# CompVis/behavior-driven-video-synthesis

Hardware: AMD Instinct MI355X
Metric: frames/sec VUnet 256x256 bs=16 fwd+bwd (higher is better)
Workload: dtype f32 (operands scaled by a power of two and split into 2 fp16 terms, 3 partial products on fp16 MFMA, fp32 accumulate; weight gradients and uncovered layers: 3 bf16 terms / 6 products, fp32-input MFMA, fp32 VALU); 1 GPU; Human3.6m shape_and_pose_net VunetAlter 256x256 per-GPU bs=16 fwd+bwd, VGG19 perceptual + KL loss, fused Adam, dropout 0.05, regressor side loop off, seeded-synthetic VGG19 weights, rasterised synthetic stickmen; global_batch=16, parallelism=dp1, conv_precision=h2, hip_streams=4, hip_graph=True, graph_settle_steps=7, rccl_world_size=1, dp_backend=none

## Files before the change

behavior_driven_video_synthesis_amd/csrc/conv_p2.hip:

```cpp
#include <stdio.h>

#include <type_traits>

#include "common.h"
#include "split_h2.h"

namespace {

constexpr int P2_META = 128, P2_AMAX0 = 16, P2_NSLOT = 64;

struct P2Args {
  const uint4* x;
  const int* xmeta;
  const uint4* w;
  const float* wk;
  const float* shift;
  const uint4* mask;
  uint4* y;
  int* ymeta;
  int N, C, H, W, M;
  int relu;
};

__device__ __forceinline__ void p2_dma(uint32_t voff, const void* sbase, uint32_t lds_addr) {
// ... 284 lines not shown
  for (size_t i = (size_t)blockIdx.x * 256 + threadIdx.x; i < total; i += (size_t)gridDim.x * 256) {
    const int xw = (int)(i % W);
    size_t t = i / W;
    const int yh = (int)(t % H);
    t /= H;
    const float* src = x + (t * 8) * HW + (size_t)yh * W + xw;
    float v[8];
#pragma unroll
    for (int j = 0; j < 8; ++j) {
      float f = src[j * HW];
      if (relu) f = f > 0.f ? f : 0.f;
      v[j] = f * s;
    }
    uint4 h, l;
    h2_split2(v[0], v[1], h.x, l.x);
    h2_split2(v[2], v[3], h.y, l.y);
    h2_split2(v[4], v[5], h.z, l.z);
    h2_split2(v[6], v[7], h.w, l.w);
    const size_t o = (t * Hp + (yh + 1)) * Wp + (xw + 1);
    y[o] = h;
    y[plane + o] = l;
  }
}
__device__ __forceinline__ void p2_unpack(const uint4& h, const uint4& l, float inv, float* v) {
  const uint32_t hs[4] = {h.x, h.y, h.z, h.w}, ls[4] = {l.x, l.y, l.z, l.w};
#pragma unroll
  for (int j = 0; j < 4; ++j) {
    const h2_f16x2 a = __builtin_bit_cast(h2_f16x2, hs[j]), b = __builtin_bit_cast(h2_f16x2, ls[j]);
    v[2 * j] = ((float)a[0] + (float)b[0] * (1.f / 2048.f)) * inv;
    v[2 * j + 1] = ((float)a[1] + (float)b[1] * (1.f / 2048.f)) * inv;
  }
}
__global__ __launch_bounds__(256) void p2_to_nchw_kernel(const uint4* __restrict__ x, const int* __restrict__ xmeta,
                                                         float* __restrict__ y, int N, int C, int H, int W) {
  const int CB = C >> 3, Hp = H + 2, Wp = W + 2;
  const float inv = h2_pow2(-xmeta[0]);
  const size_t HW = (size_t)H * W, total = (size_t)N * CB * HW, plane = (size_t)N * CB * Hp * Wp;
  for (size_t i = (size_t)blockIdx.x * 256 + threadIdx.x; i < total; i += (size_t)gridDim.x * 256) {
    const int xw = (int)(i % W);
    size_t t = i / W;
    const int yh = (int)(t % H);
    t /= H;
    const size_t o = (t * Hp + (yh + 1)) * Wp + (xw + 1);
    float v[8];
    p2_unpack(x[o], x[plane + o], inv, v);
    float* dst = y + (t * 8) * HW + (size_t)yh * W + xw;
#pragma unroll
    for (int j = 0; j < 8; ++j) dst[j * HW] = v[j];
  }
}
}

extern "C" int vunet_p2_from_nchw(const float* x, const float* amax, int32_t n_amax, int32_t relu, void* y, int32_t* ymeta,
                                  int32_t N, int32_t C, int32_t H, int32_t W, void* stream) {
  if (!x || !amax || n_amax < 1 || !y || !ymeta || C % 8 || N < 1) return VUNET_ERR_ARG;
// ... 19 lines not shown
```

behavior_driven_video_synthesis_amd/csrc/conv_thin.hip:

```cpp
#include <string.h>

#include "conv_route.h"
#include "split_h2.h"

template <int MODE>
__global__ __launch_bounds__(256) void conv_thin_m_kernel(const GatherArgs a) {
  const vunet_conv_desc& d = a.d;
  const int H = d.Hs, W = d.Ws, HW = a.HsWs;
  const int tiles_w = (W + 31) / 32, tiles_h = (H + 7) / 8;
  const unsigned bid = xcd_remap(blockIdx.x, gridDim.x);
  const int tx = bid % tiles_w;
  const int ty = (bid / tiles_w) % tiles_h;
  const int n = bid / (tiles_w * tiles_h);
  const int ow = tx * 32 + (threadIdx.x & 31), oh = ty * 8 + (threadIdx.x >> 5);
  const bool inside = ow < W && oh < H;
  int off[9];
  uint32_t ok = 0;
#pragma unroll
  for (int t = 0; t < 9; ++t) {
    const int ih = oh + t / 3 - 1, iw = ow + t % 3 - 1;
    const bool v = inside && (unsigned)ih < (unsigned)H && (unsigned)iw < (unsigned)W;
    off[t] = v ? ih * W + iw : 0;
    ok |= (v ? 1u : 0u) << t;
  }
// ... 76 lines not shown
    for (int t = 0; t < 9; ++t) {
      const int tap = MODE == 0 ? t : 8 - t;
      const float* __restrict__ w = wt + (size_t)(tap * Cp + c) * d.Mpad;
#pragma unroll
      for (int r = 0; r < R; ++r)
#pragma unroll
        for (int m = 0; m < 4; ++m) acc[r][m] = fmaf(w[m], xv[r + t / 3][t % 3], acc[r][m]);
    }
  }
  if (ow >= W) return;
  PixGeo g;
  g.n = n;
  g.ow = ow;
  g.valid = true;
#pragma unroll
  for (int r = 0; r < R; ++r) {
    g.oh = oh0 + r;
    if (g.oh < H) {
#pragma unroll
      for (int m = 0; m < 4; ++m)
        if (m < d.M) store_out(a, g, m, acc[r][m]);
    }
  }
}

template <int KS, int CI>
__global__ __launch_bounds__(256, KS == 3 ? 2 : 4) void conv_thin_k_kernel(const GatherArgs a) {
  constexpr int T = KS * KS;
  const vunet_conv_desc& d = a.d;
  const int H = d.Hs, W = d.Ws, HW = a.HsWs;
  const int tiles_w = (W + 31) / 32, tiles_h = (H + 7) / 8;
  const unsigned bid = xcd_remap(blockIdx.x, gridDim.x);
  const int tx = bid % tiles_w;
  const int ty = (bid / tiles_w) % tiles_h;
  const int n = bid / (tiles_w * tiles_h);
  const int ow = tx * 32 + (threadIdx.x & 31), oh = ty * 8 + (threadIdx.x >> 5);
  const bool inside = ow < W && oh < H;
  constexpr int C = CI, Cp = (C + 1) & ~1;
  float xv[CI][T];
  const float* __restrict__ xs = a.x1 + (size_t)n * C * HW;
#pragma unroll
  for (int t = 0; t < T; ++t) {
    const int ih = oh + (KS == 3 ? t / 3 - 1 : 0), iw = ow + (KS == 3 ? t % 3 - 1 : 0);
    const bool v = inside && (unsigned)ih < (unsigned)H && (unsigned)iw < (unsigned)W;
    const int off = v ? ih * W + iw : 0;
#pragma unroll
// ... 226 lines not shown
    else VUNET_LAUNCH((conv_thin_k_kernel<1, 3>), grid, block, 0, st, ga);
  }
  return vunet_check_launch();
}

extern "C" int vunet_p2_conv_first(const float* x, const float* amax_x, int32_t n_amax, const float* wt_f, int32_t Mpad,
                                   const float* shift, const float* wk, void* y, int32_t* ymeta, int32_t N, int32_t H, int32_t W,
                                   int32_t M, void* stream) {
  if (!x || !amax_x || n_amax < 1 || !wt_f || !wk || !y || !ymeta) return VUNET_ERR_ARG;
  if (N < 1 || M < 8 || M % 8 || M > 128 || H % 32 || W % 32 || ((uintptr_t)y & 15)) return VUNET_ERR_UNSUPPORTED;
  GatherArgs ga;
  memset(&ga, 0, sizeof(ga));
  vunet_conv_desc& d = ga.d;
  d.N = N; d.C1 = 3; d.C2 = 0; d.Hs = H; d.Ws = W; d.M = M; d.m_off = 0; d.Mpad = Mpad; d.Ho = H; d.Wo = W; d.KH = 3; d.KW = 3;
  d.stride = 1; d.pad = 1; d.mode = 0; d.out_act = ACT_RELU;
  ga.x1 = x; ga.wt = wt_f; ga.shift = shift; ga.y = reinterpret_cast<float*>(y);
  ga.NP = N * H * W; ga.HoWo = H * W; ga.HsWs = H * W;
  ga.ph = ga.pw = -1;
  P2Out po{amax_x, (int)n_amax, wk, (int*)ymeta};
  dim3 gv((unsigned)(N * (H / 32) * (W / 32)));
  VUNET_LAUNCH((conv_thin_kv_kernel<3, 4, true>), gv, dim3(256), 0, (hipStream_t)stream, ga, po);
  return vunet_check_launch();
}
```

behavior_driven_video_synthesis_amd/csrc/conv_wgrad_thin.hip:

```cpp
#include "common.h"
#include "conv_wgrad_route.h"

struct WgradThinArgs {
  vunet_wgrad_desc d;
  const float* x1;
  const float* dy;
  float* slabs;
  float* dshift;
  int Coutp, tiles_w, tiles_per_img, ntiles;
  InAct in1;
};

__global__ __launch_bounds__(256) void conv_wgrad_thin_kernel(const WgradThinArgs a_in) {
  WgradThinArgs a = a_in;
  inact_resolve(a.in1);
  constexpr int TH = 8, TW = 32, IH = TH + 2, IW = TW + 3;
  const vunet_wgrad_desc& d = a.d;
  const int C = d.C1, H = d.Hs, W = d.Ws, HW = H * W;
  const int CP = IH * IW + 1;
  extern __shared__ __attribute__((aligned(16))) float smem[];
  float* const xT = smem;
  float4* const dyT = reinterpret_cast<float4*>(smem + ((C * CP + 3) & ~3));
  const int tid = threadIdx.x;
  const int nitems = 3 * C;
  int G = 1;
  while (G < 8 && 2 * G * nitems <= 256) G *= 2;
  const int RG = TH / G;
  const int grp = tid / nitems, it = tid - grp * nitems;
  const bool worker = grp < G;
  const int kh = it / C, ci = it - kh * C;

  float acc[3][4];
#pragma unroll
  for (int kw = 0; kw < 3; ++kw)
#pragma unroll
    for (int c = 0; c < 4; ++c) acc[kw][c] = 0.f;
  float dpart[4] = {0.f, 0.f, 0.f, 0.f};
  const int sg = tid / (TW + 2), scol = tid - sg * (TW + 2);

  for (int tile = blockIdx.x; tile < a.ntiles; tile += gridDim.x) {
    const int n = tile / a.tiles_per_img, tr = tile - n * a.tiles_per_img;
    const int ty = tr / a.tiles_w, tx = tr - ty * a.tiles_w;
    const int row0 = ty * TH, col0 = tx * TW;
    __syncthreads();
    if (sg < 7) {
      const int iw = col0 - 1 + scol;
      const bool cok = (unsigned)iw < (unsigned)W;
      for (int p0 = sg; p0 < C * IH; p0 += 7 * 8) {
        float v[8];
        uint32_t idx[8];
        bool ok[8];
#pragma unroll
        for (int e = 0; e < 8; ++e) {
          const int p = p0 + 7 * e;
          const int c = p / IH, r = p - c * IH;
          const int ih = row0 - 1 + r;
          ok[e] = p < C * IH && cok && (unsigned)ih < (unsigned)H;
          idx[e] = ok[e] ? (uint32_t)((n * C + c) * HW + ih * W + iw) : 0u;
          v[e] = a.x1[idx[e]];
        }
#pragma unroll
        for (int e = 0; e < 8; ++e) {
          const int p = p0 + 7 * e;
          if (p < C * IH) {
            const int c = p / IH, r = p - c * IH;
            xT[c * CP + r * IW + scol] = ok[e] ? apply_in_act(a.in1, v[e], idx[e]) : 0.f;
          }
        }
      }
    }
    {
      const int r = tid >> 5, col = tid & 31;
      float v[4] = {0.f, 0.f, 0.f, 0.f};
#pragma unroll
      for (int co = 0; co < 4; ++co)
        if (co < d.Cout) v[co] = a.dy[(size_t)(n * d.Cout + co) * HW + (row0 + r) * W + col0 + col];
      dyT[tid] = make_float4(v[0], v[1], v[2], v[3]);
#pragma unroll
      for (int co = 0; co < 4; ++co) dpart[co] += v[co];
    }
    __syncthreads();
    if (worker) {
      for (int rr = 0; rr < RG; ++rr) {
        const int r = grp * RG + rr;
        const float* xp = xT + ci * CP + (r + kh) * IW;
        float x0 = xp[0], x1 = xp[1];
#pragma unroll 8
        for (int col = 0; col < TW; ++col) {
          const float x2 = xp[col + 2];
          const float4 g = dyT[r * TW + col];
          acc[0][0] = fmaf(g.x, x0, acc[0][0]);
          acc[0][1] = fmaf(g.y, x0, acc[0][1]);
          acc[0][2] = fmaf(g.z, x0, acc[0][2]);
          acc[0][3] = fmaf(g.w, x0, acc[0][3]);
          acc[1][0] = fmaf(g.x, x1, acc[1][0]);
          acc[1][1] = fmaf(g.y, x1, acc[1][1]);
          acc[1][2] = fmaf(g.z, x1, acc[1][2]);
          acc[1][3] = fmaf(g.w, x1, acc[1][3]);
          acc[2][0] = fmaf(g.x, x2, acc[2][0]);
          acc[2][1] = fmaf(g.y, x2, acc[2][1]);
          acc[2][2] = fmaf(g.z, x2, acc[2][2]);
          acc[2][3] = fmaf(g.w, x2, acc[2][3]);
          x0 = x1;
          x1 = x2;
        }
      }
    }
  }

  __syncthreads();
  float* const part = smem;
  if (worker) {
#pragma unroll
    for (int kw = 0; kw < 3; ++kw)
#pragma unroll
      for (int c = 0; c < 4; ++c) part[(grp * nitems + it) * 12 + kw * 4 + c] = acc[kw][c];
  }
  __syncthreads();
  const size_t K = (size_t)9 * C;
  float* slab = a.slabs + (size_t)blockIdx.x * a.Coutp * K;
  if (tid < nitems) {
#pragma unroll
    for (int kw = 0; kw < 3; ++kw)
#pragma unroll
      for (int co = 0; co < 4; ++co) {
        float t = 0.f;
        for (int g = 0; g < G; ++g) t += part[(g * nitems + tid) * 12 + kw * 4 + co];
        if (co < d.Cout) slab[(size_t)co * K + (size_t)(kh * 3 + kw) * C + ci] = t;
      }
  }
  __syncthreads();
  float* const red = smem;
#pragma unroll
  for (int co = 0; co < 4; ++co) {
    const float s_ = wave_sum(dpart[co]);
    if ((tid & 63) == 0) red[(tid >> 6) * 4 + co] = s_;
  }
  __syncthreads();
  if (tid < a.Coutp)
    a.dshift[(size_t)blockIdx.x * a.Coutp + tid] =
        (tid < 4 && tid < d.Cout) ? (red[tid] + red[4 + tid]) + (red[8 + tid] + red[12 + tid]) : 0.f;
}

bool vunet_wgrad_thin_plan(const vunet_wgrad_desc* d, WgradRoute* r) {
  if (!(d->Cout >= 1 && d->Cout <= 4 && d->KH == 3 && d->KW == 3 && d->stride == 1 && d->pad == 1 && d->C2 == 0 &&
        d->C1 >= 8 && d->C1 <= 64 && d->Ho == d->Hs && d->Wo == d->Ws && d->Hs % 8 == 0 && d->Ws % 32 == 0 &&
        (long)d->N * d->Hs * d->Ws >= 64 * 1024))
    return false;
  r->family = WGRAD_THIN;
  r->ntiles = d->N * (d->Hs / 8) * (d->Ws / 32);
  r->nslabs = r->ntiles < 512 ? r->ntiles : 512;
  return true;
}

int vunet_wgrad_thin_launch(const WgradRoute& r, const vunet_wgrad_item& it, hipStream_t st) {
  const vunet_wgrad_desc* d = &it.d;
  WgradThinArgs a;
  a.d = *d;
  a.x1 = it.x1; a.dy = it.dy; a.slabs = it.slabs; a.dshift = it.dshift;
  a.Coutp = (d->Cout + 31) / 32 * 32;
  a.tiles_w = d->Ws / 32;
  a.tiles_per_img = (d->Hs / 8) * a.tiles_w;
  a.ntiles = r.ntiles;
  a.in1 = make_inact(d->in_act, d->in_slope, d->drop_p, d->drop_seed);
  if (d->nsplit != r.nslabs) return VUNET_ERR_ARG;
  const int CP = 10 * 35 + 1;
  const size_t lds = ((size_t)((d->C1 * CP + 3) & ~3) + 4 * 256) * sizeof(float);
  if (lds > 64 * 1024 && hipFuncSetAttribute((const void*)conv_wgrad_thin_kernel, hipFuncAttributeMaxDynamicSharedMemorySize,
                                             (int)lds) != hipSuccess)
    return VUNET_ERR_LAUNCH;
  VUNET_LAUNCH(conv_wgrad_thin_kernel, dim3(d->nsplit), dim3(256), lds, st, a);
  return vunet_check_launch();
}
```

behavior_driven_video_synthesis_amd/csrc/split_h2.h:

```cpp
#pragma once
#include "common.h"

typedef _Float16 h2_f16x8 __attribute__((ext_vector_type(8)));
typedef _Float16 h2_f16x2 __attribute__((ext_vector_type(2)));
typedef uint32_t h2_u32x4 __attribute__((ext_vector_type(4)));

constexpr int H2_SLAB = 384;
constexpr int H2_AMAX_PARTS = 1024;
constexpr int H2_TOP = 14;

__host__ __device__ __forceinline__ int h2_scale_exp(float m) {
  if (!(m > 0.f) || !(m < 3.4e38f)) return 0;
  int e;
  frexpf(m, &e);
  e = H2_TOP - e;
  return e > 126 ? 126 : e;
}

__host__ __device__ __forceinline__ float h2_pow2(int e) {
  return __uint_as_float((uint32_t)(127 + e) << 23);
}

__host__ __device__ __forceinline__ void h2_pow2_pair(int etot, float& f1, float& f2) {
  const int e1 = etot < -126 ? -126 : (etot > 126 ? 126 : etot);
  f1 = h2_pow2(e1);
  f2 = h2_pow2(etot - e1);
}

__device__ __forceinline__ void h2_split2(float a, float b, uint32_t& h, uint32_t& l) {
  h2_f16x2 ph;
  ph[0] = (_Float16)a;
  ph[1] = (_Float16)b;
  h2_f16x2 pl;
  pl[0] = (_Float16)((a - (float)ph[0]) * 2048.f);
  pl[1] = (_Float16)((b - (float)ph[1]) * 2048.f);
  h = __builtin_bit_cast(uint32_t, ph);
  l = __builtin_bit_cast(uint32_t, pl);
}

__device__ __forceinline__ void h2_split2_nat(float a, float b, uint32_t& h, uint32_t& l) {
  h2_f16x2 ph, pl;
  ph[0] = (_Float16)a;
  ph[1] = (_Float16)b;
  pl[0] = (_Float16)(a - (float)ph[0]);
  pl[1] = (_Float16)(b - (float)ph[1]);
  h = __builtin_bit_cast(uint32_t, ph);
  l = __builtin_bit_cast(uint32_t, pl);
}

__device__ __forceinline__ h2_f16x8 h2_frag(uint32_t a, uint32_t b, uint32_t c, uint32_t d) {
  h2_u32x4 u = {a, b, c, d};
  return __builtin_bit_cast(h2_f16x8, u);
}

__device__ __forceinline__ void h2_dma16(const void* gsrc, uint32_t lds_addr) {
  uint32_t keep;
  asm volatile("s_mov_b32 %0, m0\n\ts_mov_b32 m0, %2\n\ts_nop 0\n\tglobal_load_lds_dwordx4 %1, off\n\ts_mov_b32 m0, %0"
               : "=&s"(keep)
               : "v"(gsrc), "s"(lds_addr)
               : "memory");
}

// ... 9 lines not shown
```

behavior_driven_video_synthesis_amd/models/imagenet_pretrained.py:

```python
from __future__ import annotations

import math

import torch
from torch import nn

from .. import ops
from ..lib.modules import Conv2d

VGG19_CFG = [64, 64, "M", 128, 128, "M", 256, 256, 256, 256, "M", 512, 512, 512, 512, "M", 512, 512, 512, 512, "M"]


class _Marker(nn.Module):

    def __init__(self, kind):
        super().__init__()
        self.kind = kind


class VGG19(nn.Module):

    def __init__(self, width_div: int = 1):
        super().__init__()
        layers, cin = [], 3
# ... 176 lines not shown
            c, h, w = st["shp"][k]
            L = len(st["shp"])
            lst[k] = ops.Planes((self.geo[0], c, h, w), self.device, meta=st["metas"][(1 if kind == "G" else 2) * L + k])
        return lst[k]

    @staticmethod
    def _weights(m):
        w = m.__dict__.get("_p2w")
        if w is None or w.weight is not m.weight:
            w = ops.P2Weights(m.weight, m.bias)
            object.__setattr__(m, "_p2w", w)
        return w

    def _first(self):
        m = self.program[0]
        stamp = (m.weight.data_ptr(), m.weight._version, m.bias._version)
        rec = m.__dict__.get("_p2first")
        if rec is None or rec[0] != stamp:
            w, b = m.weight.detach().contiguous(), m.bias.detach().contiguous()
            wt_f, wt_d, _, shift, _, _, wx_d = ops.pack_weights(w, None, b, None, None, 3, 0, 1, True)
            wk = torch.empty(4, device=w.device, dtype=torch.float32)
            work = torch.empty(2 * w.shape[0], device=w.device, dtype=torch.float32)
            ops._call("vunet_p2_weight_bound", ops._p(w), ops._p(b), int(w.shape[0]), 3, ops._p(wk), ops._p(work), ops._stream())
            rec = (stamp, wt_f, wt_d, shift, wx_d, wk)
            object.__setattr__(m, "_p2first", rec)
        return rec

    def forward(self, role, xp, targets=None, tap_weights=None):
        st = self._role(role)
        st["metas"].zero_()
        A = st["A"]
        _, wt_f, _, shift, _, wk = self._first()
        n, _, h, w = xp.shape
        amax = ops._tagged_amax(xp)
        if amax is None:
            amax = ops.absmax_partials(xp)
        ops._call("vunet_p2_conv_first", ops._p(xp), ops._p(amax), 512, ops._p(wt_f), int(wt_f.shape[1]), ops._p(shift), ops._p(wk),
                  ops._p(A[0].buf), ops._p(A[0].meta), n, h, w, A[0].shape[1], ops._stream())
        taps, losses = {}, {}
        steps = self.program[1]
        for k, step in enumerate(steps, start=1):
            if step[0] == "conv":
                ops.p2_conv(A[k - 1], self._weights(step[1]), A[k], relu=True)
                tap = step[2]
                if tap is not None:
                    taps[tap] = A[k]
                    pool_next = k < len(steps) and steps[k][0] == "pool"
                    if targets is not None and not pool_next:
                        losses[tap] = ops.p2_l1_fwd(targets[tap], A[k], tap_weights[tap])
            else:
                prev = steps[k - 2] if k >= 2 else None
                tap = prev[2] if (prev is not None and prev[0] == "conv") else None
                if targets is not None and tap is not None:
                    losses[tap] = ops.p2_pool_fwd(A[k - 1], A[k], t=targets[tap], weight=tap_weights[tap])
                else:
# ... 32 lines not shown
                k -= 1
                continue
            below = steps[k - 2] if k >= 2 else None
            if D is None:
                tap = below[2] if (below is not None and below[0] == "conv" and has(below[2])) else None
                if tap is not None:
                    D = ops.p2_l1_bwd(targets[tap], A[k - 1], None, self._grad_buf(st, "G", k - 1), tap_scale(tap, k - 1), gouts[tap])
                k -= 1
                continue
            wts = self._weights(step[1])
            if below is None:
                D = ops.p2_conv(D, wts, self._grad_buf(st, "G", 0), dgrad=True, mask=A[0])
            elif below[0] == "pool":
                D = ops.p2_conv(D, wts, self._grad_buf(st, "G", k - 1), dgrad=True)
            elif has(below[2]):
                up = ops.p2_conv(D, wts, self._grad_buf(st, "U", k - 1), dgrad=True)
                D = ops.p2_l1_bwd(targets[below[2]], A[k - 1], up, self._grad_buf(st, "G", k - 1), tap_scale(below[2], k - 1),
                                  gouts[below[2]])
            else:
                D = ops.p2_conv(D, wts, self._grad_buf(st, "G", k - 1), dgrad=True, mask=A[k - 1])
            k -= 1
        if D is None:
            return None
        _, _, wt_d, _, wx_d, _ = self._first()
        n, h, w = self.geo
        c0 = st["shp"][0][0]
        dconv = D.to_nchw()
        dx = torch.empty(n, 3, h, w, device=self.device, dtype=torch.float32)
        ops._conv_gather(ops._dgrad_desc(n, c0, h, w, 3, h, w, 3, 1, 1, wt_d.shape[1]), dconv, None, wt_d, None, None, None, dx, wx_d)
        return dx


class P2VggLoss(torch.autograd.Function):

    @staticmethod
    def forward(ctx, xp, engine, target, tap_weights, names):
        _, losses = engine.forward("p", xp, target.planes, tap_weights)
        engine.pred_generation += 1
        ctx.engine, ctx.target, ctx.tap_weights, ctx.names = engine, target, tap_weights, names
        ctx.generation, ctx.pred_generation = target.generation, engine.pred_generation
        return tuple(losses[n] for n in names)

    @staticmethod
    def backward(ctx, *gouts):
        if ctx.target.generation != ctx.generation:
            raise RuntimeError("P2VggLoss.backward: the target features were overwritten by a later target pass of the same "
                               "PerceptualVGG (its planes buffers are persistent): run forward + backward per target")
        if ctx.engine.pred_generation != ctx.pred_generation:
            raise RuntimeError("P2VggLoss.backward: a later vgg_loss() of the same PerceptualVGG and input geometry has overwritten "
                               "this pass's activations (persistent planes buffers): call backward() before the next vgg_loss(), "
                               "or switch the planes path off (models.imagenet_pretrained.enable_p2(False)) for this use")
        g = ctx.engine.backward(ctx.target.planes, ctx.tap_weights,
# ... 122 lines not shown
```

behavior_driven_video_synthesis_amd/ops.py:

```python
from __future__ import annotations

import contextlib
import ctypes
import gc
import os
from collections import namedtuple
from dataclasses import dataclass
from typing import Optional, Tuple

import torch

from . import _lib

ACT_NONE, ACT_ELU, ACT_RELU, ACT_SIGMOID, ACT_LRELU = (_lib.const("VUNET_ACT_" + a) for a in ("NONE", "ELU", "RELU", "SIGMOID", "LRELU"))
SEED2_OFFSET = 0x9E3779B9

ConvDesc = _lib.struct("vunet_conv_desc")
WgradDesc = _lib.struct("vunet_wgrad_desc")
WgradItem = _lib.struct("vunet_wgrad_item")
WnDesc = _lib.struct("vunet_wn_desc")
WnItem = _lib.struct("vunet_wn_item")
WnBwdItem = _lib.struct("vunet_wn_bwd_item")
P2Desc = _lib.struct("vunet_p2_desc")

# ... 1643 lines not shown


P2_META_INTS = 128


class Planes:

    __slots__ = ("buf", "meta", "shape")

    def __init__(self, shape, device, meta=None):
        n, c, h, w = shape
        assert c % 8 == 0
        self.shape = (int(n), int(c), int(h), int(w))
        self.buf = torch.zeros(2, n, c // 8, h + 2, w + 2, 8, device=device, dtype=torch.float16)
        self.meta = meta if meta is not None else torch.zeros(P2_META_INTS, device=device, dtype=torch.int32)

    def to_nchw(self):
        n, c, h, w = self.shape
        y = torch.empty(n, c, h, w, device=self.buf.device, dtype=torch.float32)
        _call("vunet_p2_to_nchw", _p(self.buf), _p(self.meta), _p(y), n, c, h, w, _stream())
        return y


def p2_from_nchw(x, out: Planes = None, relu: bool = False, amax=None, zero_meta: bool = True) -> Planes:
    _dev(x)
    x = _c(x)
    if out is None:
        out = Planes(tuple(x.shape), x.device)
    if amax is None:
        amax = _tagged_amax(x)
    if amax is None:
        amax = absmax_partials(x)
    n, c, h, w = x.shape
    if zero_meta:
        out.meta.zero_()
    _call("vunet_p2_from_nchw", _p(x), _p(amax), min(int(amax.numel()), 512), int(relu), _p(out.buf), _p(out.meta), n, c, h, w,
          _stream())
    return out


class P2Weights:

    def __init__(self, weight, bias):
        self.weight, self.bias = weight, bias
        self.cout, self.cin = int(weight.shape[0]), int(weight.shape[1])
        self._img = {}
# ... 75 lines not shown
```

include/vunet_hip.h:

```cpp
#ifndef VUNET_HIP_H
#define VUNET_HIP_H
#include <stddef.h>
#include <stdint.h>

#ifdef __cplusplus
extern "C" {
#endif

#define VUNET_OK 0
#define VUNET_ERR_ARG (-1)
#define VUNET_ERR_LAUNCH (-2)
#define VUNET_ERR_UNSUPPORTED (-3)

#define VUNET_ACT_NONE 0
#define VUNET_ACT_ELU 1
#define VUNET_ACT_RELU 2
#define VUNET_ACT_SIGMOID 3
#define VUNET_ACT_LRELU 4

int vunet_abi_version(void);

typedef struct vunet_conv_desc {
  int32_t N;
  int32_t C1, C2;
// ... 179 lines not shown

int vunet_adam_step(float* param, const float* grad, float* exp_avg, float* exp_avg_sq, int64_t n, float lr,
                    float beta1, float beta2, float eps, float weight_decay, int32_t step, float grad_scale,
                    void* stream);

int vunet_adam_step_dev(float* param, const float* grad, float* exp_avg, float* exp_avg_sq, int64_t n,
                        const double* lr_dev, float beta1, float beta2, float eps, float weight_decay,
                        const int64_t* step_dev, float grad_scale, void* stream);

int vunet_set_dropout_step(const uint32_t* step_dev);

#define VUNET_TUNE_SPLIT_FORCE_NT 0
#define VUNET_TUNE_TILED_FORCE_NT 1
#define VUNET_TUNE_FORCE_SMALL 2
#define VUNET_TUNE_BLK_FORCE_NT 3
#define VUNET_TUNE_PARITY_LAUNCHES 4
#define VUNET_TUNE_BLK_WS 5
#define VUNET_TUNE_WGRAD_ROWSPLIT 6
#define VUNET_TUNE_S2_FWD_F32 7
#define VUNET_TUNE_P2_FORM 8
#define VUNET_TUNE_P2_TERMS 9
#define VUNET_TUNE_COUNT 10
int vunet_set_tuning(int32_t key, int32_t value);

int vunet_dropout_mask(float* mask, int64_t n, float p, uint32_t seed, void* stream);

int vunet_stickman_raster(const float* kps, int32_t B, int32_t J, const int32_t* body, int32_t n_body,
                          const int32_t* cmds, int32_t n_cmds, uint8_t* out_u8, float* out_f32, int32_t H, int32_t W,
                          void* stream);
int vunet_stickman_raster_thick(const float* kps, int32_t B, int32_t J, const int32_t* body, int32_t n_body,
                                const int32_t* cmds, int32_t n_cmds, uint8_t* out_u8, float* out_f32, int32_t H, int32_t W,
                                int32_t thickness, void* stream);
int vunet_u8_to_unit(const uint8_t* in, float* out, int64_t n, void* stream);

int vunet_ssim_partial(const float* x, const float* y, int32_t planes, int32_t H, int32_t W, float data_range,
                       const float* window11, float* partial, void* stream);

int vunet_dp_available(void);
int vunet_dp_unique_id(void* id128);
int vunet_dp_init(int32_t world, int32_t rank, const void* id128);
int vunet_dp_world(void);
int vunet_dp_allreduce_bucket(float* buf, int64_t n, int32_t average, void* stream);
int vunet_dp_finalize(void);

int vunet_crop_window(const float* x, float* y, int32_t planes, int32_t H, int32_t W, int32_t P, const int32_t* off,
                      void* stream);
// ... 11 lines not shown

int vunet_set_schedule(double* lr_dev, double lr, float* imax_dev, float imax, int32_t* step_dev, int32_t step, void* stream);

int vunet_sum_amax(const float* const* srcs, int32_t n, float* out, float* amax_out, int64_t numel, void* stream);

typedef struct vunet_p2_desc {
  int32_t N, C, H, W;
  int32_t M;
  int32_t relu;
} vunet_p2_desc;
int vunet_p2_conv_supported(const vunet_p2_desc* d);
int vunet_p2_conv_variant(const vunet_p2_desc* d, char* name, int32_t len);
int vunet_p2_conv(const vunet_p2_desc* d, const void* x, const int32_t* xmeta, const void* w_image, const float* wk,
                  const float* shift, const void* mask, void* y, int32_t* ymeta, void* stream);
int vunet_p2_weight_image_bytes(int32_t Cout, int32_t Cin, int32_t dgrad);
int vunet_p2_pack_weights(const float* w, const float* shift, int32_t Cout, int32_t Cin, int32_t dgrad, void* image, float* wk,
                          float* workspace, void* stream);
int vunet_p2_weight_bound(const float* w, const float* shift, int32_t Cout, int32_t Cin, float* wk, float* workspace, void* stream);
int vunet_p2_conv_first(const float* x, const float* amax_x, int32_t n_amax, const float* wt_f, int32_t Mpad, const float* shift,
                        const float* wk, void* y, int32_t* ymeta, int32_t N, int32_t H, int32_t W, int32_t M, void* stream);
int vunet_p2_from_nchw(const float* x, const float* amax, int32_t n_amax, int32_t relu, void* y, int32_t* ymeta, int32_t N,
                       int32_t C, int32_t H, int32_t W, void* stream);
int vunet_p2_to_nchw(const void* x, const int32_t* xmeta, float* y, int32_t N, int32_t C, int32_t H, int32_t W, void* stream);

int vunet_p2_l1_fwd(const void* t, const int32_t* tmeta, const void* p, const int32_t* pmeta, float* partial, float* out,
                    float weight, int32_t N, int32_t C, int32_t H, int32_t W, void* stream);
int vunet_p2_pool_fwd(const void* t, const int32_t* tmeta, const void* p, const int32_t* pmeta, float* partial, float* out,
                      float weight, void* y, int32_t* ymeta, int32_t N, int32_t C, int32_t H, int32_t W, void* stream);
int vunet_p2_l1_bwd(const void* t, const int32_t* tmeta, const void* p, const int32_t* pmeta, const void* add,
                    const int32_t* addmeta, void* g, int32_t* gmeta, float gscale, const float* gout, int32_t N, int32_t C,
                    int32_t H, int32_t W, void* stream);
int vunet_p2_pool_bwd(const void* t, const int32_t* tmeta, const void* p, const int32_t* pmeta, const void* dy,
                      const int32_t* dymeta, void* g, int32_t* gmeta, float gscale, const float* gout, int32_t N, int32_t C,
                      int32_t H, int32_t W, void* stream);

typedef struct vunet_seq_linear_desc {
  int32_t B, M, K, ldx, act0, act1, nets, shared_in, S;
} vunet_seq_linear_desc;
typedef struct vunet_seq_coupling_desc {
  int32_t B, C, c1, ld_in, ld_out, Mp, reverse, affine_on_src, S;
} vunet_seq_coupling_desc;
typedef struct vunet_seq_lstm_desc {
  int32_t B, H, ldx, hoff, n, ldraw;
  int64_t seq_stride;
} vunet_seq_lstm_desc;
int vunet_seq_linear(const vunet_seq_linear_desc* d, const float* w0, const float* w1, const float* x, const float* bias0,
// ... 30 lines not shown
```

Before: 810.7 frames/s.

## Fuse p2 unpack into first-layer dgrad and prefetch thin wgrad inputs

The first VGG conv's input gradient now reads the split-fp16 plane tensor directly. A new thin kernel stages unpacked tiles in shared memory, so the separate to_nchw conversion pass and its fp32 intermediate are no longer needed. The thin weight-gradient kernel gains templated register prefetch of the next tile's input and dy values, which overlaps global loads with compute, and its launch bounds now request two blocks per SIMD. This adds register pressure and more kernel variants, and the new dgrad path is only taken when the router would have chosen the thin kernel.

```diff
diff --git a/behavior_driven_video_synthesis_amd/csrc/conv_p2.hip b/behavior_driven_video_synthesis_amd/csrc/conv_p2.hip
--- a/behavior_driven_video_synthesis_amd/csrc/conv_p2.hip
+++ b/behavior_driven_video_synthesis_amd/csrc/conv_p2.hip
@@ -330,15 +330,6 @@
     y[plane + o] = l;
   }
 }
-__device__ __forceinline__ void p2_unpack(const uint4& h, const uint4& l, float inv, float* v) {
-  const uint32_t hs[4] = {h.x, h.y, h.z, h.w}, ls[4] = {l.x, l.y, l.z, l.w};
-#pragma unroll
-  for (int j = 0; j < 4; ++j) {
-    const h2_f16x2 a = __builtin_bit_cast(h2_f16x2, hs[j]), b = __builtin_bit_cast(h2_f16x2, ls[j]);
-    v[2 * j] = ((float)a[0] + (float)b[0] * (1.f / 2048.f)) * inv;
-    v[2 * j + 1] = ((float)a[1] + (float)b[1] * (1.f / 2048.f)) * inv;
-  }
-}
 __global__ __launch_bounds__(256) void p2_to_nchw_kernel(const uint4* __restrict__ x, const int* __restrict__ xmeta,
                                                          float* __restrict__ y, int N, int C, int H, int W) {
   const int CB = C >> 3, Hp = H + 2, Wp = W + 2;
diff --git a/behavior_driven_video_synthesis_amd/csrc/conv_thin.hip b/behavior_driven_video_synthesis_amd/csrc/conv_thin.hip
--- a/behavior_driven_video_synthesis_amd/csrc/conv_thin.hip
+++ b/behavior_driven_video_synthesis_amd/csrc/conv_thin.hip
@@ -122,6 +122,97 @@
         if (m < d.M) store_out(a, g, m, acc[r][m]);
     }
   }
+}
+
+constexpr int THIN_P2_WIN = 34 * 34;
+struct ThinP2Args {
+  const uint4* x;
+  const int* xmeta;
+  const float* wt;
+  float* y;
+  int N, C, H, W, M;
+};
+template <int NM, int R>
+__global__ __launch_bounds__(256) void conv_thin_mv_p2_kernel(const ThinP2Args a) {
+  static_assert(R == 4, "a 32-row tile is 8 strips of R rows");
+  constexpr int WIN = THIN_P2_WIN, NU = (WIN + 255) / 256;
+  const int H = a.H, W = a.W, Hp = H + 2, Wp = W + 2;
+  const int tiles_w = (W + 31) / 32, tiles_h = (H + 8 * R - 1) / (8 * R);
+  const unsigned bid = xcd_remap(blockIdx.x, gridDim.x);
+  const int tx = bid % tiles_w;
+  const int ty = (bid / tiles_w) % tiles_h;
+  const int n = bid / (tiles_w * tiles_h);
+  const int j = threadIdx.x & 31, strip = threadIdx.x >> 5;
+  const int ow = tx * 32 + j, oh0 = ty * 8 * R + strip * R;
+  const int CB = a.C >> 3;
+  const float inv = h2_pow2(-a.xmeta[0]);
+  const size_t plane = (size_t)a.N * CB * Hp * Wp;
+  __shared__ float xs[8 * WIN];
+  uint32_t uoff[NU], uok = 0;
+#pragma unroll
+  for (int i = 0; i < NU; ++i) {
+    const int u = threadIdx.x + i * 256;
+    const int pr = ty * 32 + u / 34, pc = tx * 32 + u % 34;
+    const bool ok = u < WIN && pr < Hp && pc < Wp;
+    uoff[i] = ok ? (uint32_t)(pr * Wp + pc) : 0u;
+    uok |= (ok ? 1u : 0u) << i;
+  }
+  uint4 uh[NU], ul[NU];
+  auto fetch = [&](int cb, int i) {
+    const uint4* __restrict__ src = a.x + ((size_t)n * CB + cb) * Hp * Wp;
+    uh[i] = src[uoff[i]];
+    ul[i] = src[plane + uoff[i]];
+  };
+  float acc[R][NM];
+#pragma unroll
+  for (int r = 0; r < R; ++r)
+#pragma unroll
+    for (int m = 0; m < NM; ++m) acc[r][m] = 0.f;
+  const float* __restrict__ wt = a.wt;
+  const float* __restrict__ xl = xs + strip * R * 34 + j;
+#pragma unroll
+  for (int i = 0; i < NU; ++i) fetch(0, i);
+  for (int cb = 0; cb < CB; ++cb) {
+#pragma unroll
+    for (int i = 0; i < NU; ++i) {
+      const int u = threadIdx.x + i * 256;
+      if (u < WIN) {
+        float v[8];
+        p2_unpack(uh[i], ul[i], inv, v);
+#pragma unroll
+        for (int c = 0; c < 8; ++c) xs[c * WIN + u] = ((uok >> i) & 1u) ? v[c] : 0.f;
+      }
+      if (cb + 1 < CB) fetch(cb + 1, i);
+    }
+    __syncthreads();
+#pragma unroll 2
+    for (int cc = 0; cc < 8; ++cc) {
+      const int c = cb * 8 + cc;
+      float xv[R + 2][3];
+#pragma unroll
+      for (int r = 0; r < R + 2; ++r)
+#pragma unroll
+        for (int k = 0; k < 3; ++k) xv[r][k] = xl[cc * WIN + r * 34 + k];
+#pragma unroll
+      for (int t = 0; t < 9; ++t) {
+        const float* __restrict__ w = wt + c * 36 + (8 - t) * 4;
+#pragma unroll
+        for (int r = 0; r < R; ++r)
+#pragma unroll
+          for (int m = 0; m < NM; ++m) acc[r][m] = fmaf(w[m], xv[r + t / 3][t % 3], acc[r][m]);
+      }
+    }
+    __syncthreads();
+  }
+  if (ow >= W) return;
+  const size_t HW = (size_t)H * W;
+#pragma unroll
+  for (int r = 0; r < R; ++r)
+    if (oh0 + r < H) {
+#pragma unroll
+      for (int m = 0; m < NM; ++m)
+        if (m < a.M) a.y[((size_t)n * a.M + m) * HW + (size_t)(oh0 + r) * W + ow] = acc[r][m];
+    }
 }
 
 template <int KS, int CI>
@@ -394,3 +485,33 @@
   VUNET_LAUNCH((conv_thin_kv_kernel<3, 4, true>), gv, dim3(256), 0, (hipStream_t)stream, ga, po);
   return vunet_check_launch();
 }
+
+extern "C" int vunet_p2_dgrad_first(const void* x, const int32_t* xmeta, const float* wc, float* y, int32_t N, int32_t C,
+                                    int32_t H, int32_t W, int32_t M, void* stream) {
+  if (!x || !xmeta || !wc || !y) return VUNET_ERR_ARG;
+  if (N < 1 || H < 1 || W < 1 || C < 8 || C % 8 || M < 1 || M > 4 || ((uintptr_t)x & 15) || ((uintptr_t)wc & 15))
+    return VUNET_ERR_UNSUPPORTED;
+  const int64_t tiles = (int64_t)N * ((H + 31) / 32) * ((W + 31) / 32);
+  if ((int64_t)N * C * (H + 2) * (W + 2) >= (1ll << 31) || tiles >= (1ll << 31)) return VUNET_ERR_UNSUPPORTED;
+  const ThinP2Args a{(const uint4*)x, (const int*)xmeta, wc, y, (int)N, (int)C, (int)H, (int)W, (int)M};
+  dim3 gv((unsigned)tiles);
+  if (M == 4) VUNET_LAUNCH((conv_thin_mv_p2_kernel<4, 4>), gv, dim3(256), 0, (hipStream_t)stream, a);
+  else VUNET_LAUNCH((conv_thin_mv_p2_kernel<3, 4>), gv, dim3(256), 0, (hipStream_t)stream, a);
+  return vunet_check_launch();
+}
+
+extern "C" int vunet_conv_thin_dgrad_strips(const float* x, const float* wt_d, int32_t Mpad, float* y, int32_t N, int32_t C,
+                                            int32_t H, int32_t W, int32_t M, void* stream) {
+  if (!x || !wt_d || !y) return VUNET_ERR_ARG;
+  if (N < 1 || H < 1 || W < 1 || C < 1 || M < 1 || M > 4 || Mpad < 32 || Mpad % 32) return VUNET_ERR_UNSUPPORTED;
+  const int64_t tiles = (int64_t)N * ((H + 31) / 32) * ((W + 31) / 32);
+  if ((int64_t)N * C * H * W >= (1ll << 31)) return VUNET_ERR_UNSUPPORTED;
+  vunet_conv_desc d;
+  memset(&d, 0, sizeof(d));
+  d.N = N; d.C1 = C; d.Hs = H; d.Ws = W; d.M = M; d.Mpad = Mpad; d.Ho = H; d.Wo = W; d.KH = 3; d.KW = 3;
+  d.stride = 1; d.pad = 1; d.mode = 1;
+  GatherArgs ga;
+  fill_gather_args(ga, &d, x, nullptr, wt_d, nullptr, nullptr, nullptr, nullptr, y, false);
+  VUNET_LAUNCH((conv_thin_mv_kernel<1, 4>), dim3((unsigned)tiles), dim3(256), 0, (hipStream_t)stream, ga);
+  return vunet_check_launch();
+}
diff --git a/behavior_driven_video_synthesis_amd/csrc/conv_wgrad_thin.hip b/behavior_driven_video_synthesis_amd/csrc/conv_wgrad_thin.hip
--- a/behavior_driven_video_synthesis_amd/csrc/conv_wgrad_thin.hip
+++ b/behavior_driven_video_synthesis_amd/csrc/conv_wgrad_thin.hip
@@ -1,3 +1,5 @@
+#include <type_traits>
+
 #include "common.h"
 #include "conv_wgrad_route.h"
 
@@ -11,9 +13,50 @@
   InAct in1;
 };
 
-__global__ __launch_bounds__(256) void conv_wgrad_thin_kernel(const WgradThinArgs a_in) {
+__device__ __forceinline__ void wgrad_thin_finish(const WgradThinArgs& a, float* smem, const float (&acc)[3][4],
+                                                  const float (&dpart)[4], int G, int nitems, int grp, int it, int kh, int ci,
+                                                  bool worker) {
+  const vunet_wgrad_desc& d = a.d;
+  const int C = d.C1, tid = threadIdx.x;
+  __syncthreads();
+  float* const part = smem;
+  if (worker) {
+#pragma unroll
+    for (int kw = 0; kw < 3; ++kw)
+#pragma unroll
+      for (int c = 0; c < 4; ++c) part[(grp * nitems + it) * 12 + kw * 4 + c] = acc[kw][c];
+  }
+  __syncthreads();
+  const size_t K = (size_t)9 * C;
+  float* slab = a.slabs + (size_t)blockIdx.x * a.Coutp * K;
+  if (tid < nitems) {
+#pragma unroll
+    for (int kw = 0; kw < 3; ++kw)
+#pragma unroll
+      for (int co = 0; co < 4; ++co) {
+        float t = 0.f;
+        for (int g = 0; g < G; ++g) t += part[(g * nitems + tid) * 12 + kw * 4 + co];
+        if (co < d.Cout) slab[(size_t)co * K + (size_t)(kh * 3 + kw) * C + ci] = t;
+      }
+  }
+  __syncthreads();
+  float* const red = smem;
+#pragma unroll
+  for (int co = 0; co < 4; ++co) {
+    const float s_ = wave_sum(dpart[co]);
+    if ((tid & 63) == 0) red[(tid >> 6) * 4 + co] = s_;
+  }
+  __syncthreads();
+  if (tid < a.Coutp)
+    a.dshift[(size_t)blockIdx.x * a.Coutp + tid] =
+        (tid < 4 && tid < d.Cout) ? (red[tid] + red[4 + tid]) + (red[8 + tid] + red[12 + tid]) : 0.f;
+}
+
+template <int NL>
+__global__ __launch_bounds__(256, 2) void conv_wgrad_thin_kernel(const WgradThinArgs a_in) {
   WgradThinArgs a = a_in;
   inact_resolve(a.in1);
+  const int in_form = in_act_form_of(a.in1);
   constexpr int TH = 8, TW = 32, IH = TH + 2, IW = TW + 3;
   const vunet_wgrad_desc& d = a.d;
   const int C = d.C1, H = d.Hs, W = d.Ws, HW = H * W;
@@ -38,48 +81,106 @@
   float dpart[4] = {0.f, 0.f, 0.f, 0.f};
   const int sg = tid / (TW + 2), scol = tid - sg * (TW + 2);
 
+  auto line = [&](int k, int n, int row0, int col0, uint32_t& idx) -> bool {
+    const int c = sg + 7 * (k / IH), r = k % IH;
+    const int ih = row0 - 1 + r, iw = col0 - 1 + scol;
+    const bool ok = c < C && (unsigned)iw < (unsigned)W && (unsigned)ih < (unsigned)H;
+    idx = ok ? (uint32_t)((n * C + c) * HW + ih * W + iw) : 0u;
+    return ok;
+  };
+  float xr[NL > 0 ? NL : 1], dyr[4];
+  auto fetch = [&](int tile) {
+    const int n = tile / a.tiles_per_img, tr = tile - n * a.tiles_per_img;
+    const int ty = tr / a.tiles_w, tx = tr - ty * a.tiles_w;
+    const int row0 = ty * TH, col0 = tx * TW;
+    if (sg < 7) {
+      const int iw = min(max(col0 - 1 + scol, 0), W - 1);
+#pragma unroll
+      for (int k = 0; k < NL; ++k) {
+        const int c = min(sg + 7 * (k / IH), C - 1), ih = min(max(row0 - 1 + k % IH, 0), H - 1);
+        xr[k] = a.x1[(uint32_t)((n * C + c) * HW + ih * W + iw)];
+      }
+    }
+    const int r = tid >> 5, col = tid & 31;
+#pragma unroll
+    for (int co = 0; co < 4; ++co)
+      dyr[co] = a.dy[(size_t)(n * d.Cout + (co < d.Cout ? co : 0)) * HW + (row0 + r) * W + col0 + col];
+  };
+  if constexpr (NL > 0)
+    if ((int)blockIdx.x < a.ntiles) fetch(blockIdx.x);
+
   for (int tile = blockIdx.x; tile < a.ntiles; tile += gridDim.x) {
     const int n = tile / a.tiles_per_img, tr = tile - n * a.tiles_per_img;
     const int ty = tr / a.tiles_w, tx = tr - ty * a.tiles_w;
     const int row0 = ty * TH, col0 = tx * TW;
     __syncthreads();
-    if (sg < 7) {
-      const int iw = col0 - 1 + scol;
-      const bool cok = (unsigned)iw < (unsigned)W;
-      for (int p0 = sg; p0 < C * IH; p0 += 7 * 8) {
-        float v[8];
-        uint32_t idx[8];
-        bool ok[8];
-#pragma unroll
-        for (int e = 0; e < 8; ++e) {
-          const int p = p0 + 7 * e;
-          const int c = p / IH, r = p - c * IH;
-          const int ih = row0 - 1 + r;
-          ok[e] = p < C * IH && cok && (unsigned)ih < (unsigned)H;
-          idx[e] = ok[e] ? (uint32_t)((n * C + c) * HW + ih * W + iw) : 0u;
-          v[e] = a.x1[idx[e]];
-        }
-#pragma unroll
-        for (int e = 0; e < 8; ++e) {
-          const int p = p0 + 7 * e;
-          if (p < C * IH) {
+    if constexpr (NL > 0) {
+      auto put = [&](auto form) {
+#pragma unroll
+        for (int k = 0; k < NL; ++k) {
+          const int c = sg + 7 * (k / IH), r = k % IH;
+          if (c < C) {
+            uint32_t idx;
+            const bool ok = line(k, n, row0, col0, idx);
+            xT[c * CP + r * IW + scol] = ok ? in_act_form<decltype(form)::value>(a.in1, xr[k], idx) : 0.f;
+          }
+        }
+      };
+      if (sg < 7) {
+        switch (in_form) {
+          case 0: put(std::integral_constant<int, 0>{}); break;
+          case 1: put(std::integral_constant<int, 1>{}); break;
+          case 2: put(std::integral_constant<int, 2>{}); break;
+          default: put(std::integral_constant<int, 3>{}); break;
+        }
+      }
+#pragma unroll
+      for (int co = 0; co < 4; ++co) {
+        if (co >= d.Cout) dyr[co] = 0.f;
+        dpart[co] += dyr[co];
+      }
+      dyT[tid] = make_float4(dyr[0], dyr[1], dyr[2], dyr[3]);
+    } else {
+      if (sg < 7) {
+        const int iw = col0 - 1 + scol;
+        const bool cok = (unsigned)iw < (unsigned)W;
+        for (int p0 = sg; p0 < C * IH; p0 += 7 * 8) {
+          float v[8];
+          uint32_t idx[8];
+          bool ok[8];
+#pragma unroll
+          for (int e = 0; e < 8; ++e) {
+            const int p = p0 + 7 * e;
             const int c = p / IH, r = p - c * IH;
-            xT[c * CP + r * IW + scol] = ok[e] ? apply_in_act(a.in1, v[e], idx[e]) : 0.f;
+            const int ih = row0 - 1 + r;
+            ok[e] = p < C * IH && cok && (unsigned)ih < (unsigned)H;
+            idx[e] = ok[e] ? (uint32_t)((n * C + c) * HW + ih * W + iw) : 0u;
+            v[e] = a.x1[idx[e]];
           }
-        }
-      }
-    }
-    {
-      const int r = tid >> 5, col = tid & 31;
-      float v[4] = {0.f, 0.f, 0.f, 0.f};
-#pragma unroll
-      for (int co = 0; co < 4; ++co)
-        if (co < d.Cout) v[co] = a.dy[(size_t)(n * d.Cout + co) * HW + (row0 + r) * W + col0 + col];
-      dyT[tid] = make_float4(v[0], v[1], v[2], v[3]);
-#pragma unroll
-      for (int co = 0; co < 4; ++co) dpart[co] += v[co];
+#pragma unroll
+          for (int e = 0; e < 8; ++e) {
+            const int p = p0 + 7 * e;
+            if (p < C * IH) {
+              const int c = p / IH, r = p - c * IH;
+              xT[c * CP + r * IW + scol] = ok[e] ? apply_in_act(a.in1, v[e], idx[e]) : 0.f;
+            }
+          }
+        }
+      }
+      {
+        const int r = tid >> 5, col = tid & 31;
+        float v[4] = {0.f, 0.f, 0.f, 0.f};
+#pragma unroll
+        for (int co = 0; co < 4; ++co)
+          if (co < d.Cout) v[co] = a.dy[(size_t)(n * d.Cout + co) * HW + (row0 + r) * W + col0 + col];
+        dyT[tid] = make_float4(v[0], v[1], v[2], v[3]);
+#pragma unroll
+        for (int co = 0; co < 4; ++co) dpart[co] += v[co];
+      }
     }
     __syncthreads();
+    if constexpr (NL > 0)
+      if (tile + (int)gridDim.x < a.ntiles) fetch(tile + gridDim.x);
     if (worker) {
       for (int rr = 0; rr < RG; ++rr) {
         const int r = grp * RG + rr;
@@ -108,39 +209,10 @@
     }
   }
 
-  __syncthreads();
-  float* const part = smem;
-  if (worker) {
-#pragma unroll
-    for (int kw = 0; kw < 3; ++kw)
-#pragma unroll
-      for (int c = 0; c < 4; ++c) part[(grp * nitems + it) * 12 + kw * 4 + c] = acc[kw][c];
-  }
-  __syncthreads();
-  const size_t K = (size_t)9 * C;
-  float* slab = a.slabs + (size_t)blockIdx.x * a.Coutp * K;
-  if (tid < nitems) {
-#pragma unroll
-    for (int kw = 0; kw < 3; ++kw)
-#pragma unroll
-      for (int co = 0; co < 4; ++co) {
-        float t = 0.f;
-        for (int g = 0; g < G; ++g) t += part[(g * nitems + tid) * 12 + kw * 4 + co];
-        if (co < d.Cout) slab[(size_t)co * K + (size_t)(kh * 3 + kw) * C + ci] = t;
-      }
-  }
-  __syncthreads();
-  float* const red = smem;
-#pragma unroll
-  for (int co = 0; co < 4; ++co) {
-    const float s_ = wave_sum(dpart[co]);
-    if ((tid & 63) == 0) red[(tid >> 6) * 4 + co] = s_;
-  }
-  __syncthreads();
-  if (tid < a.Coutp)
-    a.dshift[(size_t)blockIdx.x * a.Coutp + tid] =
-        (tid < 4 && tid < d.Cout) ? (red[tid] + red[4 + tid]) + (red[8 + tid] + red[12 + tid]) : 0.f;
-}
+  wgrad_thin_finish(a, smem, acc, dpart, G, nitems, grp, it, kh, ci, worker);
+}
+
+static int g_wgrad_thin_form = 0;
 
 bool vunet_wgrad_thin_plan(const vunet_wgrad_desc* d, WgradRoute* r) {
   if (!(d->Cout >= 1 && d->Cout <= 4 && d->KH == 3 && d->KW == 3 && d->stride == 1 && d->pad == 1 && d->C2 == 0 &&
@@ -166,9 +238,19 @@
   if (d->nsplit != r.nslabs) return VUNET_ERR_ARG;
   const int CP = 10 * 35 + 1;
   const size_t lds = ((size_t)((d->C1 * CP + 3) & ~3) + 4 * 256) * sizeof(float);
-  if (lds > 64 * 1024 && hipFuncSetAttribute((const void*)conv_wgrad_thin_kernel, hipFuncAttributeMaxDynamicSharedMemorySize,
+  if (lds > 64 * 1024 && hipFuncSetAttribute((const void*)conv_wgrad_thin_kernel<0>, hipFuncAttributeMaxDynamicSharedMemorySize,
                                              (int)lds) != hipSuccess)
     return VUNET_ERR_LAUNCH;
-  VUNET_LAUNCH(conv_wgrad_thin_kernel, dim3(d->nsplit), dim3(256), lds, st, a);
+  const int nl = g_wgrad_thin_form == 1 || d->C1 > 35 ? 0 : 10 * ((d->C1 + 6) / 7);
+  if (nl == 0) VUNET_LAUNCH(conv_wgrad_thin_kernel<0>, dim3(d->nsplit), dim3(256), lds, st, a);
+  else if (nl <= 20) VUNET_LAUNCH(conv_wgrad_thin_kernel<20>, dim3(d->nsplit), dim3(256), lds, st, a);
+  else if (nl <= 30) VUNET_LAUNCH(conv_wgrad_thin_kernel<30>, dim3(d->nsplit), dim3(256), lds, st, a);
+  else VUNET_LAUNCH(conv_wgrad_thin_kernel<50>, dim3(d->nsplit), dim3(256), lds, st, a);
   return vunet_check_launch();
 }
+
+extern "C" int vunet_wgrad_thin_set_form(int32_t form) {
+  if (form != 0 && form != 1) return VUNET_ERR_ARG;
+  g_wgrad_thin_form = form;
+  return VUNET_OK;
+}
diff --git a/behavior_driven_video_synthesis_amd/csrc/split_h2.h b/behavior_driven_video_synthesis_amd/csrc/split_h2.h
--- a/behavior_driven_video_synthesis_amd/csrc/split_h2.h
+++ b/behavior_driven_video_synthesis_amd/csrc/split_h2.h
@@ -38,6 +38,16 @@
   l = __builtin_bit_cast(uint32_t, pl);
 }
 
+__device__ __forceinline__ void p2_unpack(const uint4& h, const uint4& l, float inv, float* v) {
+  const uint32_t hs[4] = {h.x, h.y, h.z, h.w}, ls[4] = {l.x, l.y, l.z, l.w};
+#pragma unroll
+  for (int j = 0; j < 4; ++j) {
+    const h2_f16x2 a = __builtin_bit_cast(h2_f16x2, hs[j]), b = __builtin_bit_cast(h2_f16x2, ls[j]);
+    v[2 * j] = ((float)a[0] + (float)b[0] * (1.f / 2048.f)) * inv;
+    v[2 * j + 1] = ((float)a[1] + (float)b[1] * (1.f / 2048.f)) * inv;
+  }
+}
+
 __device__ __forceinline__ void h2_split2_nat(float a, float b, uint32_t& h, uint32_t& l) {
   h2_f16x2 ph, pl;
   ph[0] = (_Float16)a;
diff --git a/behavior_driven_video_synthesis_amd/models/imagenet_pretrained.py b/behavior_driven_video_synthesis_amd/models/imagenet_pretrained.py
--- a/behavior_driven_video_synthesis_amd/models/imagenet_pretrained.py
+++ b/behavior_driven_video_synthesis_amd/models/imagenet_pretrained.py
@@ -1,5 +1,6 @@
 from __future__ import annotations
 
+import ctypes
 import math
 
 import torch
@@ -222,7 +223,7 @@
             wk = torch.empty(4, device=w.device, dtype=torch.float32)
             work = torch.empty(2 * w.shape[0], device=w.device, dtype=torch.float32)
             ops._call("vunet_p2_weight_bound", ops._p(w), ops._p(b), int(w.shape[0]), 3, ops._p(wk), ops._p(work), ops._stream())
-            rec = (stamp, wt_f, wt_d, shift, wx_d, wk)
+            rec = (stamp, wt_f, wt_d, shift, wx_d, wk, ops.p2_dgrad_first_weights(wt_d, int(w.shape[0])))
             object.__setattr__(m, "_p2first", rec)
         return rec
 
@@ -230,7 +231,7 @@
         st = self._role(role)
         st["metas"].zero_()
         A = st["A"]
-        _, wt_f, _, shift, _, wk = self._first()
+        _, wt_f, _, shift, _, wk, _ = self._first()
         n, _, h, w = xp.shape
         amax = ops._tagged_amax(xp)
         if amax is None:
@@ -309,12 +310,18 @@
             k -= 1
         if D is None:
             return None
-        _, _, wt_d, _, wx_d, _ = self._first()
+        _, _, wt_d, _, wx_d, _, wc_d = self._first()
         n, h, w = self.geo
         c0 = st["shp"][0][0]
+        desc = ops._dgrad_desc(n, c0, h, w, 3, h, w, 3, 1, 1, wt_d.shape[1])
+        if ops._kernel_name("vunet_conv2d_variant", ctypes.byref(desc), 0, ops._scheme() if wx_d is not None else 0,
+                            0).startswith("conv_thin_mv_kernel"):
+            dx = ops.p2_dgrad_first(D, wc_d, 3)
+            if dx is not None:
+                return dx
         dconv = D.to_nchw()
         dx = torch.empty(n, 3, h, w, device=self.device, dtype=torch.float32)
-        ops._conv_gather(ops._dgrad_desc(n, c0, h, w, 3, h, w, 3, 1, 1, wt_d.shape[1]), dconv, None, wt_d, None, None, None, dx, wx_d)
+        ops._conv_gather(desc, dconv, None, wt_d, None, None, None, dx, wx_d)
         return dx
 
 
diff --git a/behavior_driven_video_synthesis_amd/ops.py b/behavior_driven_video_synthesis_amd/ops.py
--- a/behavior_driven_video_synthesis_amd/ops.py
+++ b/behavior_driven_video_synthesis_amd/ops.py
@@ -1689,6 +1689,22 @@
         return y
 
 
+def p2_dgrad_first_weights(wt_d, c: int):
+    return wt_d.view(9, -1, wt_d.shape[1])[:, :c, :4].permute(1, 0, 2).contiguous()
+
+
+def p2_dgrad_first(x: Planes, wc, m: int):
+    n, c, h, w = x.shape
+    assert tuple(wc.shape) == (c, 9, 4) and wc.is_contiguous()
+    y = torch.empty(n, m, h, w, device=x.buf.device, dtype=torch.float32)
+    rc = _lib.lib().vunet_p2_dgrad_first(_p(x.buf), _p(x.meta), _p(wc), _p(y), n, c, h, w, int(m), _stream())
+    if rc == -3:
+        return None
+    if rc != 0:
+        raise RuntimeError(f"vunet_p2_dgrad_first failed with code {rc}")
+    return y
+
+
 def p2_from_nchw(x, out: Planes = None, relu: bool = False, amax=None, zero_meta: bool = True) -> Planes:
     _dev(x)
     x = _c(x)
diff --git a/include/vunet_hip.h b/include/vunet_hip.h
--- a/include/vunet_hip.h
+++ b/include/vunet_hip.h
@@ -225,6 +225,7 @@
 #define VUNET_TUNE_P2_TERMS 9
 #define VUNET_TUNE_COUNT 10
 int vunet_set_tuning(int32_t key, int32_t value);
+int vunet_wgrad_thin_set_form(int32_t form);
 
 int vunet_dropout_mask(float* mask, int64_t n, float p, uint32_t seed, void* stream);
 
@@ -282,6 +283,10 @@
 int vunet_p2_from_nchw(const float* x, const float* amax, int32_t n_amax, int32_t relu, void* y, int32_t* ymeta, int32_t N,
                        int32_t C, int32_t H, int32_t W, void* stream);
 int vunet_p2_to_nchw(const void* x, const int32_t* xmeta, float* y, int32_t N, int32_t C, int32_t H, int32_t W, void* stream);
+int vunet_p2_dgrad_first(const void* x, const int32_t* xmeta, const float* wc, float* y, int32_t N, int32_t C, int32_t H,
+                         int32_t W, int32_t M, void* stream);
+int vunet_conv_thin_dgrad_strips(const float* x, const float* wt_d, int32_t Mpad, float* y, int32_t N, int32_t C, int32_t H,
+                                 int32_t W, int32_t M, void* stream);
 
 int vunet_p2_l1_fwd(const void* t, const int32_t* tmeta, const void* p, const int32_t* pmeta, float* partial, float* out,
                     float weight, int32_t N, int32_t C, int32_t H, int32_t W, void* stream);
```

Result: no change. 815.5 frames/s, median of 6 (+0.6%).
